# JWally/jsLPSolver

Hardware: AMD Instinct MI355X
Metric: simplex pivots/sec (higher is better)
Workload: dtype f64

## Files before the change

jslpsolver_amd/csrc/jslp_resident_pipe.hip.h:

```cpp
#pragma once

#ifdef JSLP_CHAOS_BUILD
#undef RT_MARK
#define RT_MARK(p)                                                                                                        \
    do {                                                                                                                  \
        if (F_TEST_LATE >= 2) {                                                                                     \
            const unsigned who_ = (R.epoch * 7u + (unsigned)(p) * 3u) % (unsigned)(THREADS / 64);                         \
            if (__builtin_amdgcn_readfirstlane((int)((unsigned)(threadIdx.x >> 6) == who_))) __builtin_amdgcn_s_sleep(100); \
            if (F_TEST_LATE >= 3 && (R.epoch + (unsigned)(p)) % 5u == (unsigned)blockIdx.x % 5u) __builtin_amdgcn_s_sleep(60); \
        }                                                                                                                 \
    } while (0)
#endif
#ifndef JSLP_PIPE_ROW_CHECKSUM
#define JSLP_PIPE_ROW_CHECKSUM 1
#endif
#ifndef JSLP_PIPE_K_BROADCAST
#define JSLP_PIPE_K_BROADCAST 1
#endif
#ifndef JSLP_PIPE_NORM_PUB
#define JSLP_PIPE_NORM_PUB 1
#endif
#ifndef JSLP_PIPE_ROW_CHECKSUM_MAXCPT
#define JSLP_PIPE_ROW_CHECKSUM_MAXCPT 4
#endif
#define JSLP_CK_K32(k) ((0x9E3779B1u * (unsigned)(2 * (k) + 1)) | 0x80000001u)
#define JSLP_CK_PAIR(CK, LO, HI, j)                                                                                               \
    do {                                                                                                                          \
        (CK) += (u64_t)(unsigned)(LO) * JSLP_CK_K32(2 * (j)) + (u64_t)(unsigned)((LO) >> 32) * JSLP_CK_K32(2 * (j) + 1);           \
        (CK) += (u64_t)(unsigned)(HI) * JSLP_CK_K32(2 * (j) + 2) + (u64_t)(unsigned)((HI) >> 32) * JSLP_CK_K32(2 * (j) + 3);       \
    } while (0)
#define JSLP_CK_TAGMIX(tag) ((u64_t)(tag) * 0xD6E8FEB86659FD93ull)
#ifndef JSLP_PIPE_POLL_MISSING_ONLY
#define JSLP_PIPE_POLL_MISSING_ONLY 1
#endif
#ifndef JSLP_PIPE_S_VIA_LDS
#define JSLP_PIPE_S_VIA_LDS 1
#endif
#define JSLP_PUB_SKEW 256
#ifndef JSLP_G16_STRIDE
#define JSLP_G16_STRIDE 64
#endif
#define JSLP_PIPE_KCHUNK 8

#define JSLP_HOST_ABORT_PERIOD 1024u
#ifndef JSLP_HOST_ABORT
#define JSLP_HOST_ABORT 1
#endif
#define JSLP_HOST_ABORT_FORCE_RETRY(SPINS) (JSLP_HOST_ABORT && (SPINS) == 0u && (epoch & (JSLP_HOST_ABORT_PERIOD - 1u)) == JSLP_HOST_ABORT_PERIOD - 1u && b == f.G - 1 && wv == HAWV)
#define JSLP_HOST_ABORT_IN_SPIN(SPINS, SWEPT)                                                                                     \
    if (JSLP_HOST_ABORT && (SPINS) == 1u && (epoch & (JSLP_HOST_ABORT_PERIOD - 1u)) == JSLP_HOST_ABORT_PERIOD - 1u && b == f.G - 1 && wv == HAWV) { \
        const unsigned* ha_ = *reinterpret_cast<const unsigned* const*>(reinterpret_cast<const char*>(f.cdev) + sizeof(Ctx));     \
        if (ha_ != nullptr && __hip_atomic_load(ha_, __ATOMIC_RELAXED, __HIP_MEMORY_SCOPE_SYSTEM) != 0u) {  \
            if (lane == 0) AG_STORE(f.abort_flag, 1u);                                                                            \
            (SWEPT) = false;                                                                                                      \
            break;                                                                                                                \
        }                                                                                                                         \
    }

__device__ __forceinline__ double readlane_f64(double x, int src_lane) {
    const long long b = __double_as_longlong(x);
    const unsigned lo = (unsigned)__builtin_amdgcn_readlane((int)(unsigned)b, src_lane);
    const unsigned hi = (unsigned)__builtin_amdgcn_readlane((int)(unsigned)((unsigned long long)b >> 32), src_lane);
    return __longlong_as_double((long long)(((unsigned long long)hi << 32) | lo));
}


static_assert(offsetof(RSmem, cycbits_tail) == offsetof(RSmem, lhist) + sizeof(int2) * JSLP_R_LHIST, "the filter runs from inside lhist into cycbits_tail");
static_assert((JSLP_R_LHIST - JSLP_PIPE_LHIST) * 8 + JSLP_R_CYCEXTRA * 4 == JSLP_PIPE_CYCBITS / 8, "filter size");
__device__ __forceinline__ unsigned* cyc_bits(RSmem& sm) { return reinterpret_cast<unsigned*>(&sm.lhist[JSLP_PIPE_LHIST]); }
__device__ __forceinline__ int cyc_pair_seen(RSmem& sm, int2 pair) {
    static_assert(JSLP_PIPE_CYCBITS == (1 << 19), "the hashes below yield 19 bits");
    unsigned* bits = cyc_bits(sm);
    const unsigned k = (unsigned)pair.x * 0x9E3779B1u ^ (unsigned)pair.y * 0x85EBCA6Bu;
    const unsigned h1 = k >> (32 - 19), h2 = (k * 0xC2B2AE35u + 0x27D4EB2Fu) >> (32 - 19);
    const unsigned o1 = bits[h1 >> 5], m1 = 1u << (h1 & 31u);
    bits[h1 >> 5] = o1 | m1;
    const unsigned o2 = bits[h2 >> 5], m2 = 1u << (h2 & 31u);
    bits[h2 >> 5] = o2 | m2;
    return ((o1 & m1) != 0u && (o2 & m2) != 0u) ? 1 : 0;
}
__device__ __forceinline__ bool cyc_suffix_is_square(const int2* lds, const int2* glob, int n, int2 last, Smem& red) {
    auto at = [&](int i) -> int2 { return i < JSLP_PIPE_LHIST ? lds[i] : glob[i]; };
    int found = 0;
    for (int L = 1 + threadIdx.x; 2 * L <= n; L += blockDim.x) {
        const int2 a = at(n - 1 - L);
        if (a.x != last.x || a.y != last.y) continue;
        bool eq = true;
        for (int i = 0; i < L - 1; i++) {
            const int2 x = at(n - 2 * L + i), y = at(n - L + i);
            if (x.x != y.x || x.y != y.y) { eq = false; break; }
        }
        if (eq) found = 1;
    }
    (void)red;
    return __syncthreads_or(found) != 0;
}

#define JSLP_WAVE_FOLD32(X, OP, ID)                                                                                              \
    do {                                                                                                                         \
        X = OP(X, __builtin_amdgcn_update_dpp((int)(ID), X, 0xB1, 0xf, 0xf, false));                                             \
        X = OP(X, __builtin_amdgcn_update_dpp((int)(ID), X, 0x4E, 0xf, 0xf, false));                                             \
        X = OP(X, __builtin_amdgcn_update_dpp((int)(ID), X, 0x141, 0xf, 0xf, false));                                            \
        X = OP(X, __builtin_amdgcn_update_dpp((int)(ID), X, 0x140, 0xf, 0xf, false));                                            \
        X = OP(X, __builtin_amdgcn_update_dpp((int)(ID), X, 0x142, 0xa, 0xf, false));                                            \
        X = OP(X, __builtin_amdgcn_update_dpp((int)(ID), X, 0x143, 0xc, 0xf, false));                                            \
        X = __builtin_amdgcn_readlane(X, 63);                                                                                    \
    } while (0)
__device__ __forceinline__ int jslp_add_i32(int a, int b) { return (int)((unsigned)a + (unsigned)b); }
__device__ __forceinline__ u64_t u64_wave_add_halves(u64_t x) {
    int lo = (int)(unsigned)x, hi = (int)(unsigned)(x >> 32);
    JSLP_WAVE_FOLD32(lo, jslp_add_i32, 0);
    JSLP_WAVE_FOLD32(hi, jslp_add_i32, 0);
    return (u64_t)(unsigned)lo | ((u64_t)(unsigned)hi << 32);
}
#define JSLP_CK_WAVE(CK) u64_wave_add_halves((CK) * (u64_t)(unsigned)(2 * tid + 1))

static_assert(offsetof(RSmem, part_r) % 8 == 0 && JSLP_F_MAXG / 64 >= 2, "winner and verdict are one aligned 8-byte word");
template <int CPT, int ROWS>
struct PipeDiet {
    static constexpr bool ONE_BARRIER = ROWS <= 8 && CPT <= 4;
    static constexpr bool RAW_ATOMICS = ROWS <= 8 && CPT <= 4;
};

__device__ __forceinline__ unsigned lds_offset(const void* p) { return (unsigned)(size_t)(__attribute__((address_space(3))) const void*)p; }
__device__ __forceinline__ void lds_max_u64_raw(u64_t* p, u64_t v) { asm volatile("ds_max_u64 %0, %1" : : "v"(lds_offset(p)), "v"(v) : "memory"); }
__device__ __forceinline__ void lds_min_i32_raw(int32_t* p, int v) { asm volatile("ds_min_i32 %0, %1" : : "v"(lds_offset(p)), "v"(v) : "memory"); }
__device__ __forceinline__ void lds_raw_drain() { asm volatile("s_waitcnt lgkmcnt(0)" : : : "memory"); }
template <bool ONE>
__device__ __forceinline__ void gather_post(RSmem& sm, int winner, bool swept) {
    if (ONE) *reinterpret_cast<int2*>(&sm.part_r[0]) = make_int2(winner, swept ? 1 : 0);
    else sm.part_r[0] = winner;
}
template <bool ONE>
__device__ __forceinline__ bool gather_close(RSmem& sm, bool swept, int* winner) {
    if (ONE) {
        __syncthreads();
        const int2 v = *reinterpret_cast<const int2*>(&sm.part_r[0]);
        *winner = v.x;
        return v.y != 0;
    }
    const bool ok = __syncthreads_and(swept ? 1 : 0) != 0;
    *winner = sm.part_r[0];
    return ok;
}

template <int THREADS, int CPT, bool UNR, bool RAW>
__device__ __forceinline__ int price_row_pipe(const double (&x)[CPT], int c0, const int (&pb)[CPT], const Ctx& c, RSmem& sm, int par,
                                              double* value, unsigned unr, int* neg, bool* claim) {
    const int tid = threadIdx.x, lane = tid & 63, wv = tid >> 6;
    double bv = c.precision;
    int bi = 0, bb = 0, bneg = 0;
#pragma unroll
    for (int j = 0; j < CPT; j++) {
        const int col = c0 + j;
        const bool isneg = UNR && ((unr >> j) & 1u) && x[j] < 0;
        const double val = isneg ? -x[j] : x[j];
        const bool ok = col >= 1 && col < c.W && val > c.precision;
        const bool take = ok && (bi == 0 || pb[j] < bb || (pb[j] == bb && val > bv));
        bv = take ? val : bv;
        bi = take ? col : bi;
        bb = take ? pb[j] : bb;
        bneg = take ? (isneg ? 1 : 0) : bneg;
    }
    {
        const unsigned long long m = __ballot(bi != 0);
        if (m != 0ull) {
            const int first = __ffsll((long long)m) - 1;
            const int wave_b = __builtin_amdgcn_readlane(bb, first);
            if (lane == 0) { if (RAW) lds_min_i32_raw(&sm.pw_batch[par], wave_b); else atomicMin(&sm.pw_batch[par], wave_b); }
        }
    }
    if (RAW) lds_raw_drain();
    __syncthreads();
    const int wb = sm.pw_batch[par];
    if (tid == THREADS - 1) { sm.pw_batch[par ^ 1] = 0x7fffffff; sm.pw_val[par ^ 1] = 0; sm.pw_col[par ^ 1] = 0x7fffffff; }
    *claim = false;
    if (wb == 0x7fffffff) return 0;
    const u64_t bits = (u64_t)__double_as_longlong(bv);
    const bool cand = bi != 0 && bb == wb;
    if (cand) { if (RAW) lds_max_u64_raw(&sm.pw_val[par], bits); else atomicMax(&sm.pw_val[par], bits); }
    if (RAW) lds_raw_drain();
    __syncthreads();
    const u64_t wvv = sm.pw_val[par];
    if (cand && bits == wvv) { if (RAW) lds_min_i32_raw(&sm.pw_col[par], bi); else atomicMin(&sm.pw_col[par], bi); }
    if (RAW) lds_raw_drain();
    __syncthreads();
    const int pcol = sm.pw_col[par];
    double v = __longlong_as_double((long long)wvv);
    if (UNR) {
        if (cand && bi == pcol) sm.pw_neg[par] = bneg;
        __syncthreads();
        *neg = sm.pw_neg[par];
        if (*neg) v = -v;
    }
    *value = v;
    *claim = wv == ((pcol / CPT) >> 6);
    return pcol;
}

#define JSLP_R_MAXOPT 3

template <int CPT>
__device__ __forceinline__ int price_optional_regs(const double (&x)[CPT], const double (&oo)[JSLP_R_MAXOPT][CPT], int c0, const Ctx& c, RSmem& sm) {
    const double precision = c.precision;
    for (int o = 0; o < c.n_opt && o < JSLP_R_MAXOPT; o++) {
        Cand best; best.v = precision; best.i = 0; best.b = 0;
#pragma unroll
        for (int j = 0; j < CPT; j++) {
            const int col = c0 + j;
            if (col < 1 || col >= c.W) continue;
            bool deferred = -precision < x[j] && x[j] < precision;
#pragma unroll
            for (int q = 0; q < JSLP_R_MAXOPT; q++) {
                if (q > o || !deferred) break;
                const double v = oo[q][j];
                if (q < o) { deferred = -precision < v && v < precision; continue; }
                if (-precision < v && v < precision) break;
                const bool take = v > best.v;
                best.v = take ? v : best.v;
                best.i = take ? col : best.i;
            }
        }
        const Cand e = block_reduce(best, PriceFirst(), sm.f.red);
        if (e.i != 0) return e.i;
    }
    return 0;
}

#define JSLP_PIPE_UPDATE_ROW(i)                                                                             \
    do {                                                                                                    \
        const int r_ = r_begin + (i);                                                                       \
        if (r_ >= r_end) break;                                                                             \
        if (r_ == 0) {                                                \
            _Pragma("unroll") for (int j = 0; j < CPT; j++) a[i][j] = r0[j];                                \
            break;                                                                                          \
        }                                                                                                   \
        if (r_ == pr_p) {                                                                                   \
            _Pragma("unroll") for (int j = 0; j < CPT; j++) a[i][j] = p[j];                                 \
            break;                                                                                          \
        }                                                                                                   \
        const double ki_ = kis[i];                                                                          \
        if (nonzero16(ki_)) {                                                                               \
            _Pragma("unroll") for (int j = 0; j < CPT; j++)                                                 \
                if ((nzm >> j) & 1u) a[i][j] = eliminate(a[i][j], ki_, p[j]);                               \
            if (has_pc_p) {                                                                                 \
                const double nv_ = sm.nv[i];                                                                \
                _Pragma("unroll") for (int j = 0; j < CPT; j++)                                             \
                    if (pc_p == c0 + j) a[i][j] = nv_;                                                      \
            }                                                                                               \
        }                                                                                                   \
    } while (0)

template <int CPT, int ROWS, bool OPT, bool XL>
struct PipeUpd {
    static constexpr bool UFAST = !XL && !OPT && ROWS <= 8 && CPT <= 4;
    static constexpr bool PUBTREE = UFAST && ROWS == 8;
    static constexpr unsigned ALL_ROWS = (unsigned)((1ull << ROWS) - 1ull);
    static __device__ __forceinline__ unsigned dead_rows(int live) { return ALL_ROWS & ~(unsigned)((1ull << max(0, min(ROWS, live))) - 1ull); }
};
#define JSLP_OPAQUE_SGPR(x) ({ int o_ = (x); asm volatile("" : "+s"(o_)); o_; })
#define JSLP_XL_UPDATE_PASS()                                                                                                     \
    do {                                                                                                                          \
                                                                                              \
        const double kl_ = lane < ROWS ? sm.colb[par_p][lane] : 0.0;                                                              \
        const unsigned km_ = (unsigned)__ballot(nonzero16(kl_));    \
         \
        if (UFAST) {                                                                                                              \
                  \
            double kb_[ROWS];                                                                                                     \
            _Pragma("unroll") for (int i = 0; i < ROWS; i++) kb_[i] = sm.colb[par_p][i];                                          \
            const int om_ = (int)(km_ | dead_rows), full_ = (int)ALL_ROWS;                                                        \
            if (om_ == full_) {                                                                                                   \
                _Pragma("unroll") for (int j = 0; j < CPT; j++) {                                                                 \
                    if ((nzm >> j) & 1u) {                                                                                        \
                        _Pragma("unroll") for (int i = 0; i < ROWS; i++) a[i][j] = eliminate(a[i][j], kb_[i], p[j]);              \
                    }                                                                                                             \
                }                                                                                                                 \
            }                                                                                                                     \
            if (JSLP_OPAQUE_SGPR(om_) != full_) {                                                                                 \
                _Pragma("unroll") for (int j = 0; j < CPT; j++) {                                                                 \
                    if ((nzm >> j) & 1u) {                                                                                        \
                        _Pragma("unroll") for (int i = 0; i < ROWS; i++)                                                          \
                            if (km_ & (1u << i)) a[i][j] = eliminate(a[i][j], kb_[i], p[j]);                                      \
                    }                                                                                                             \
                }                                                                                                                 \
            }                                                                                                                     \
        } else if (JSLP_PIPE_K_BROADCAST) {                                                                                       \
            _Pragma("unroll") for (int i0 = 0; i0 < ROWS; i0 += 8) {                                                              \
                double kb_[8];                                                                                                    \
                _Pragma("unroll") for (int i = 0; i < 8; i++) kb_[i] = (i0 + i < ROWS) ? sm.colb[par_p][i0 + i] : 0.0;            \
                _Pragma("unroll") for (int j = 0; j < CPT; j++) {                                                                 \
                    if ((nzm >> j) & 1u) {                                                                                        \
                        _Pragma("unroll") for (int i = 0; i < 8; i++)                                                             \
                            if (i0 + i < ROWS && (km_ & (1u << (i0 + i)))) a[i0 + i][j] = eliminate(a[i0 + i][j], kb_[i], p[j]);  \
                    }                                                                                                             \
                }                                                                                                                 \
            }                                                                                                                     \
        } else {                                                                                                                  \
        _Pragma("unroll") for (int j = 0; j < CPT; j++) {                                                                         \
            if ((nzm >> j) & 1u) {                                                                                                \
                _Pragma("unroll") for (int i = 0; i < ROWS; i++)                                                                  \
                    if (km_ & (1u << i)) a[i][j] = eliminate(a[i][j], readlane_f64(kl_, i), p[j]);                                \
            }                                                                                                                     \
        }                                                                                                                         \
        }                                                                                                                         \
        if (wv == ((pc_p / CPT) >> 6)) {          \
            const int ol_ = __builtin_amdgcn_readfirstlane((pc_p / CPT) & 63), js_ = __builtin_amdgcn_readfirstlane(pc_p % CPT);  \
             \
            const double nvl_ = lane < ROWS ? (NPUB ? -kl_ / quot_p : sm.nv[lane]) : 0.0;                                         \
            _Pragma("unroll") for (int j = 0; j < CPT; j++)                                                                       \
                if (js_ == j) {                                                                                                   \
                    _Pragma("unroll") for (int i = 0; i < ROWS; i++)                                                              \
                        if (km_ & (1u << i)) { const double nv_ = readlane_f64(nvl_, i); if (lane == ol_) a[i][j] = nv_; }        \
                }                                                                                                                 \
        }                                                                                                                         \
        {                                                                 \
            const int ip_ = __builtin_amdgcn_readfirstlane(pr_p - r_begin);                                                       \
            if (ip_ >= 0 && ip_ < ROWS) {                                                                                         \
                _Pragma("unroll") for (int i = 0; i < ROWS; i++)                                                                  \
                    if (i == JSLP_OPAQUE_SGPR(ip_)) { _Pragma("unroll") for (int j = 0; j < CPT; j++) a[i][j] = p[j]; }           \
            }                                                                                                                     \
        }                                                                                                                         \
        if (b == 0) { _Pragma("unroll") for (int j = 0; j < CPT; j++) a[0][j] = r0[j]; }    \
    } while (0)
#define JSLP_XL_PUBLISH_ROW(ROW)                                                                                                  \
    do {                                                                                                                          \
        const int ipub_ = __builtin_amdgcn_readfirstlane((ROW) - r_begin);                                                        \
        if (colok) {                                                                                                              \
            _Pragma("unroll") for (int i = 0; i < ROWS; i++)                                                                      \
                if (i == JSLP_OPAQUE_SGPR(ipub_)) {                                                                                                 \
                    const int off_ = par * pub_stride + (b * ld + c0) * 16;                                                       \
                    _Pragma("unroll") for (int j = 0; j < CPT; j++) {                                                             \
                        if (c0 + j >= ld) continue;                                                                               \
                        const u64_t d_ = (u64_t)__double_as_longlong(a[i][j]);                                                    \
                        v4u_t v_;                                                                                                 \
                        v_.x = (unsigned)d_; v_.y = tag; v_.z = (unsigned)(d_ >> 32); v_.w = tag;                                 \
                        __builtin_amdgcn_raw_buffer_store_b128(v_, rsrc_rows, off_ + j * 16, 0, ST_AUX);                          \
                    }                                                                                                             \
                }                                                                                                                 \
        }                                                                                                                         \
    } while (0)
#define JSLP_PUB_COPY(i) do { _Pragma("unroll") for (int j = 0; j < CPT; j++) { double t_ = a[i][j]; asm volatile("" : "+v"(t_)); cand_[j] = t_; } } while (0)
#define JSLP_PUBLISH_ROW_PLAIN(ROW)                                                                                               \
    do {                                                                                                                          \
        const int ipub_ = __builtin_amdgcn_readfirstlane((ROW) - r_begin);                                                        \
                     \
        const bool flag_first_ = CKS && __builtin_amdgcn_readfirstlane((int)(F_TEST_LATE == 2 && wv == 0)) != 0;                  \
        const bool torn_ = CKS && __builtin_amdgcn_readfirstlane((int)((F_TEST_LATE == 4 || F_TEST_LATE == 6) && wv == 0)) != 0;  \
        const bool early_lane_ = !torn_ || ((lane & 1) == (F_TEST_LATE == 6 ? 1 : 0));                                            \
        u64_t ck_ = 0;                                                                                                            \
        double cand_[CPT];                      \
        _Pragma("unroll") for (int j = 0; j < CPT; j++) cand_[j] = 0.0;                                                           \
        if (PUBTREE) {  \
            if (JSLP_OPAQUE_SGPR(ipub_) < 4) {                                                                                    \
                if (JSLP_OPAQUE_SGPR(ipub_) < 2) { if (JSLP_OPAQUE_SGPR(ipub_) == 0) JSLP_PUB_COPY(0); else if (JSLP_OPAQUE_SGPR(ipub_) == 1) JSLP_PUB_COPY(1); } \
                else { if (JSLP_OPAQUE_SGPR(ipub_) == 2) JSLP_PUB_COPY(2); else if (JSLP_OPAQUE_SGPR(ipub_) == 3) JSLP_PUB_COPY(3); } \
            } else {                                                                                                              \
                if (JSLP_OPAQUE_SGPR(ipub_) < 6) { if (JSLP_OPAQUE_SGPR(ipub_) == 4) JSLP_PUB_COPY(4); else if (JSLP_OPAQUE_SGPR(ipub_) == 5) JSLP_PUB_COPY(5); } \
                else { if (JSLP_OPAQUE_SGPR(ipub_) == 6) JSLP_PUB_COPY(6); else if (JSLP_OPAQUE_SGPR(ipub_) == 7) JSLP_PUB_COPY(7); } \
            }                                                                                                                     \
        } else                                                                                                                    \
        _Pragma("unroll") for (int i = 0; i < ROWS; i++)                                                                          \
            if (i == JSLP_OPAQUE_SGPR(ipub_)) {  \
                _Pragma("unroll") for (int j = 0; j < CPT; j++) { double t_ = a[i][j]; asm volatile("" : "+v"(t_)); cand_[j] = t_; }               \
            }                                                                                                                     \
        double quotc_ = 0.0, nv0c_ = 0.0;                                                                                         \
        if (NPUB) {                                                                                                               \
                         \
            quotc_ = sm.colb[par][ipub_];                                                                                         \
                                               \
            const bool holds_pc_ = __builtin_amdgcn_readfirstlane((int)(wv == ((pub_pc / CPT) >> 6))) != 0;                       \
            double rq_ = 0.0;                                                                                                     \
            if (holds_pc_) { rq_ = 1.0 / quotc_; nv0c_ = -pub_k0 / quotc_; }                                                      \
            _Pragma("unroll") for (int j = 0; j < CPT; j++) {                                                                     \
                const int col_ = c0 + j;                                                                                          \
                const double val_ = cand_[j];                                                                                     \
                double v_ = 0.0;                                                                                                  \
                if (col_ < W) {                                                                                                   \
                    const bool innz_ = nonzero16(val_);                                                                           \
                    v_ = innz_ ? val_ / quotc_ : 0.0;                                                                             \
                    if (col_ == pub_pc) v_ = rq_;                                                                                 \
                    if (innz_ && !nonzero16(v_) && v_ != 0.0) v_ = 0.0;  \
                }                                                                                                                 \
                cand_[j] = v_;                                                                                                    \
            }                                                                                                                     \
        }                                                                                                                         \
        const int off_ = PERM ? par * pub_stride + b * SLOT + lane_off : par * pub_stride + (b * ld + c0) * 8;                    \
        if (colok) {                                                                                                              \
            _Pragma("unroll") for (int j = 0; j < CPT; j += 2) {                                                                  \
                if (c0 + j >= ld) continue;                                                                                       \
                const u64_t lo_ = (u64_t)__double_as_longlong(cand_[j]), hi_ = (u64_t)__double_as_longlong(cand_[j + 1]);         \
                v4u_t v_;                                                                                                         \
                v_.x = (unsigned)lo_; v_.y = (unsigned)(lo_ >> 32); v_.z = (unsigned)hi_; v_.w = (unsigned)(hi_ >> 32);           \
                if (!flag_first_ && early_lane_) __builtin_amdgcn_raw_buffer_store_b128(v_, rsrc_rows, off_ + (j >> 1) * PAIR_STEP, 0, ST_AUX); \
                if (CKS) JSLP_CK_PAIR(ck_, lo_, hi_, j);                                                                          \
            }                                                                                                                     \
        }                                                                                                                         \
        if (CKS) { if (NPUB) JSLP_CKS_RAISE_REC(ck_, quotc_, nv0c_); else JSLP_CKS_RAISE_FLAG(ck_); }                              \
        if (flag_first_ || torn_) {                                                                                               \
            __builtin_amdgcn_s_sleep(127);                                                                                        \
            if (colok && (flag_first_ || !early_lane_)) {                                                                         \
                _Pragma("unroll") for (int j = 0; j < CPT; j += 2) {                                                              \
                    if (c0 + j >= ld) continue;                                                                                   \
                    const u64_t lo_ = (u64_t)__double_as_longlong(cand_[j]), hi_ = (u64_t)__double_as_longlong(cand_[j + 1]);     \
                    v4u_t v_;                                                                                                     \
                    v_.x = (unsigned)lo_; v_.y = (unsigned)(lo_ >> 32); v_.z = (unsigned)hi_; v_.w = (unsigned)(hi_ >> 32);       \
                    __builtin_amdgcn_raw_buffer_store_b128(v_, rsrc_rows, off_ + (j >> 1) * PAIR_STEP, 0, ST_AUX);                \
                }                                                                                                                 \
            }                                                                                                                     \
        }                                                                                                                         \
    } while (0)
#define JSLP_CKS_RAISE_FLAG(CK)                                                                                                   \
    do {                                                                                                                          \
        const u64_t x_ = JSLP_CK_WAVE(CK) ^ JSLP_CK_TAGMIX(tag);                                                                  \
        if (lane == 0) AG_STORE(f.rowflagc[par] + wv * JSLP_F_MAXG + b, x_);                                                      \
    } while (0)
#define JSLP_CK_QMIX(Q, NV) (((u64_t)__double_as_longlong(Q) * 0x9E3779B97F4A7C15ull) ^ ((u64_t)__double_as_longlong(NV) * 0xC2B2AE3D27D4EB4Full))
#define JSLP_REC_OFF(PAR, WV, B) (JSLP_R_REC_OFF + (((PAR) * JSLP_R_FLAGCOPIES + (WV)) * JSLP_F_MAXG + (B)) * JSLP_R_REC_BYTES)
#define JSLP_CKS_RAISE_REC(CK, Q, NV)                                                                                             \
    do {                                                                                                                          \
        const u64_t x_ = JSLP_CK_WAVE(CK) ^ JSLP_CK_TAGMIX(tag) ^ JSLP_CK_QMIX(Q, NV);                                            \
        if (lane == 0) {                                                                                                          \
            const u64_t qb_ = (u64_t)__double_as_longlong(Q), nb_ = (u64_t)__double_as_longlong(NV);                              \
            v4u_t r0_, r1_;                                                                                                       \
            r0_.x = (unsigned)x_; r0_.y = (unsigned)(x_ >> 32); r0_.z = (unsigned)qb_; r0_.w = (unsigned)(qb_ >> 32);             \
            r1_.x = (unsigned)nb_; r1_.y = (unsigned)(nb_ >> 32); r1_.z = tag; r1_.w = 0u;                                        \
            __builtin_amdgcn_raw_buffer_store_b128(r0_, rsrc_g16, JSLP_REC_OFF(par, wv, b), 0, ST_AUX);                           \
            __builtin_amdgcn_raw_buffer_store_b128(r1_, rsrc_g16, JSLP_REC_OFF(par, wv, b) + 16, 0, ST_AUX);                      \
        }                                                                                                                         \
    } while (0)
#define JSLP_CKS_ISSUE_LOOK()                                                                                                     \
    do {                                                                                                                          \
        if (__builtin_amdgcn_readfirstlane((int)((F_TEST_LATE & 1) != 0 && wv == 0))) __builtin_amdgcn_s_sleep(127);              \
        if (NPUB) {                                     \
            rec0_ = __builtin_amdgcn_raw_buffer_load_b128(rsrc_g16, JSLP_REC_OFF(par, wv, bw), 0, 16);                            \
            rec1_ = __builtin_amdgcn_raw_buffer_load_b128(rsrc_g16, JSLP_REC_OFF(par, wv, bw) + 16, 0, 16);                       \
        } else {                                                                                                                  \
            flag_ = AG_LOAD(f.rowflagc[par] + wv * JSLP_F_MAXG + bw);                                                             \
        }                                                                                                                         \
    } while (0)
#define JSLP_CKS_FETCH_ROW()                                                                                                      \
    do {                                                                                                                          \
        efetch += 1;                                                                                                              \
        unsigned spins_ = 0;                                                                                                      \
        const u64_t tmix_ = JSLP_CK_TAGMIX(tag);                                                                                  \
        u64_t flag_ = 0;                                                                                                          \
        v4u_t rec0_, rec1_;                                                                                                       \
        rec0_.x = rec0_.y = rec0_.z = rec0_.w = 0u; rec1_ = rec0_;                                                                \
        for (;;) {                                                                                                                \
            JSLP_CKS_ISSUE_LOOK();     \
            u64_t qm_ = 0;                                                                                                        \
            u64_t ck_ = 0;                                                                                                        \
            if (colok) {                                                                                                          \
                _Pragma("unroll") for (int j = 0; j < CPT; j += 2) {                                                              \
                    if (c0 + j >= ld) continue;                                                                                   \
                    const v4u_t v_ = __builtin_amdgcn_raw_buffer_load_b128(rsrc_rows, off_in + (j >> 1) * PAIR_STEP, 0, 16);  \
                    const u64_t lo_ = (u64_t)v_.x | ((u64_t)v_.y << 32), hi_ = (u64_t)v_.z | ((u64_t)v_.w << 32);                 \
                    pv[j] = __longlong_as_double((long long)lo_);                                                                 \
                    pv[j + 1] = __longlong_as_double((long long)hi_);                                                             \
                    JSLP_CK_PAIR(ck_, lo_, hi_, j);                                                           \
                }                                                                                                                 \
            }                                                                                                                     \
            if (NPUB) {                                                                                                           \
                flag_ = (u64_t)rec0_.x | ((u64_t)rec0_.y << 32);                                                                  \
                fq = __longlong_as_double((long long)((u64_t)rec0_.z | ((u64_t)rec0_.w << 32)));                                  \
                fnv = __longlong_as_double((long long)((u64_t)rec1_.x | ((u64_t)rec1_.y << 32)));                                 \
                qm_ = JSLP_CK_QMIX(fq, fnv);                                                                                      \
            }                                                                                                                     \
            const u64_t x_ = JSLP_CK_WAVE(ck_) ^ tmix_ ^ qm_;                                                                     \
            if (__builtin_amdgcn_readfirstlane((int)(x_ == flag_))) break;                                                        \
            JSLP_RT_RETRY();                                                                                                      \
            if (lane == 0) atomicAdd(f.abort_flag + 1, 1u);  \
            __builtin_amdgcn_s_sleep(1);                                                                                          \
            ++spins_;                                                                                                             \
            bool dead_ = false;                                                                                                   \
            if ((spins_ & 63u) == 0 && AG_LOAD(f.abort_flag) != 0u) dead_ = true;                                                 \
            if (spins_ > F_SPIN) { if (lane == 0) AG_STORE(f.abort_flag, 1u); dead_ = true; }                                     \
            if (dead_) { if (lane == 0) atomicMax(&sm.okbad, efetch); break; }                                                    \
        }                                                                                                                         \
    } while (0)
#ifdef JSLP_DEBUG_RESIDENT
#define JSLP_RT_RETRY() do { if (tid == 0) R.rt_retries += 1; } while (0)
#else
#define JSLP_RT_RETRY() do { } while (0)
#endif
#define JSLP_XL_FETCH_ROW(PCCOL, QUOT)                                                                                            \
    do {                                                                                                                          \
        efetch += 1;                                                                                                              \
        unsigned spins_ = 0;                                                                                                      \
        const int off_ = par * pub_stride + (bw * ld + c0) * 16;                                                                  \
        const int offq_ = par * pub_stride + (bw * ld + (PCCOL)) * 16;       \
        for (;;) {                                                                                                                \
            if (__builtin_amdgcn_readfirstlane((int)(F_TEST_LATE != 0 && wv == 0))) __builtin_amdgcn_s_sleep(127);          \
            bool ok_ = true;                                                                                                      \
            if (colok) {                                                                                                          \
                _Pragma("unroll") for (int j = 0; j < CPT; j++) {                                                                 \
                    if (c0 + j >= ld) continue;                                                                                   \
                    const v4u_t v_ = __builtin_amdgcn_raw_buffer_load_b128(rsrc_rows, off_ + j * 16, 0, 16);                      \
                    ok_ = ok_ && v_.y == tag && v_.w == tag;                                                                      \
                    pv[j] = __longlong_as_double((long long)((u64_t)v_.x | ((u64_t)v_.z << 32)));                                 \
                }                                                                                                                 \
            }                                                                                                                     \
            if ((PCCOL) > 0) {                                                                                                    \
                const v4u_t q_ = __builtin_amdgcn_raw_buffer_load_b128(rsrc_rows, offq_, 0, 16);                                  \
                ok_ = ok_ && q_.y == tag && q_.w == tag;                                                                          \
                (QUOT) = __longlong_as_double((long long)((u64_t)q_.x | ((u64_t)q_.z << 32)));                                    \
            }                                                                                                                     \
            if (__all(ok_)) break;                                                                                                \
            __builtin_amdgcn_s_sleep(1);                                                                                          \
            ++spins_;                                                                                                             \
            bool dead_ = false;                                                                                                   \
            if ((spins_ & 63u) == 0 && AG_LOAD(f.abort_flag) != 0u) dead_ = true;                                                 \
            if (spins_ > F_SPIN) { if (lane == 0) AG_STORE(f.abort_flag, 1u); dead_ = true; }                               \
            if (dead_) { if (lane == 0) atomicMax(&sm.okbad, efetch); break; }                                                    \
        }                                                                                                                         \
    } while (0)

#define JSLP_PIPE_COMMIT_GLOBAL_NOW()                                                                                             \
    do {                                                                                                                          \
        const Ctx& g_ = *f.cdev;                                                                                                  \
        g_.vibr[pr] = entering;                                                                                                   \
        g_.vibc[pc] = leaving;                                                                                                    \
        g_.rbv[entering] = pr;                                                                                                    \
        g_.rbv[leaving] = -1;                                                                                                     \
        g_.cbv[entering] = -1;                                                                                                    \
        g_.cbv[leaving] = pc;                                                                                                     \
        if (R.trace_n < g_.trace_cap) g_.trace[R.trace_n] = make_int2(pr, pc);                                                    \
    } while (0)
#define JSLP_PIPE_HIST_GLOBAL(PAIR)                                                                                               \
    do {                                                                                                                          \
        jslp_gi32_t* const h_ = (jslp_gi32_t*)jslp_uniform_ptr(sm.gp_hist) + 2 * R.hist_n;                                        \
        h_[0] = (PAIR).x; h_[1] = (PAIR).y;                                                                                       \
    } while (0)
#define JSLP_PIPE_SWAP_LDS_MAPS()                                                                                                 \
    do {                                                                                                                          \
        if (lpend && tid == THREADS - 64) {                                                                                       \
            const int leaving_ = sm.lvibr[pr_p], entering_ = sm.lvibc[pc_p];                                                      \
            sm.lvibr[pr_p] = entering_;                                                                                           \
            sm.lvibc[pc_p] = leaving_;                                                                                            \
            if (b == 0) { sm.cm_ent = entering_; sm.cm_leav = leaving_; }                                                         \
        }                                                                                                                         \
        lpend = false;                                                                                                            \
    } while (0)
__device__ __forceinline__ void* jslp_uniform_ptr(const void* p) {
    const unsigned long long b = (unsigned long long)p;
    const unsigned lo = (unsigned)__builtin_amdgcn_readfirstlane((int)(unsigned)b), hi = (unsigned)__builtin_amdgcn_readfirstlane((int)(unsigned)(b >> 32));
    return (void*)(((unsigned long long)hi << 32) | lo);
}
typedef __attribute__((address_space(1))) int32_t jslp_gi32_t;
#define JSLP_PIPE_COMMIT_GLOBAL()                                                                                                 \
    do {                                                                                                                          \
        if (cpend && tid == THREADS - 64 && b == 0) {                                                                             \
            const int ent_ = sm.cm_ent, leav_ = sm.cm_leav;  \
             \
            jslp_gi32_t* const vibr_ = (jslp_gi32_t*)jslp_uniform_ptr(sm.gp_vibr);                                               \
            jslp_gi32_t* const vibc_ = (jslp_gi32_t*)jslp_uniform_ptr(sm.gp_vibc);                                               \
            jslp_gi32_t* const rbv_ = (jslp_gi32_t*)jslp_uniform_ptr(sm.gp_rbv);                                                 \
            jslp_gi32_t* const cbv_ = (jslp_gi32_t*)jslp_uniform_ptr(sm.gp_cbv);                                                 \
            vibr_[pr_p] = ent_;                                                                                                   \
            vibc_[pc_p] = leav_;                                                                                                  \
            rbv_[ent_] = pr_p;                                                                                                    \
            rbv_[leav_] = -1;                                                                                                     \
            cbv_[ent_] = -1;                                                                                                      \
            cbv_[leav_] = pc_p;                                                                                                   \
            if (R.trace_n - 1 < sm.gp_trace_cap) {                                                                                \
                jslp_gi32_t* const tr_ = (jslp_gi32_t*)jslp_uniform_ptr(sm.gp_trace) + 2 * (R.trace_n - 1);                       \
                tr_[0] = pr_p; tr_[1] = pc_p;                                                                                     \
            }                                                                                                                     \
        }                                                                                                                         \
        cpend = false;                                                                                                            \
    } while (0)

template <int THREADS, int CPT, int ROWS, bool OPT, bool CHK, bool XL = false, bool UNR = false>
__device__ __forceinline__ void resident_phase2_pipe(const ResCtx& f, RSmem& sm, ResRegs<CPT, ROWS>& R, int it1_start, int it2_start,
                                                     const int (&pb)[CPT]) {
    const Ctx& c = f.c;
    const int tid = threadIdx.x, b = XL ? (int)(blockIdx.x / JSLP_XL_SPREAD) : (int)blockIdx.x, lane = tid & 63, wv = tid >> 6;
    constexpr int ST_AUX = XL ? 0 : 16;
    constexpr bool TAGGED = XL;
    constexpr bool CKS = !TAGGED && JSLP_PIPE_ROW_CHECKSUM != 0 && CPT <= JSLP_PIPE_ROW_CHECKSUM_MAXCPT;
    constexpr bool NPUB = CKS && !OPT && !XL && CPT <= 4 && ROWS <= 8 && JSLP_PIPE_NORM_PUB != 0;
    constexpr bool QDIRECT = TAGGED || NPUB;
    constexpr bool ONE_FOLD = ROWS <= 8 && CPT <= 4;
    constexpr bool S_LDS = XL || JSLP_PIPE_S_VIA_LDS != 0;
    constexpr bool UPD_NEW = XL || (CPT <= 4 && !(OPT && ROWS > 8));
    typedef PipeUpd<CPT, ROWS, OPT, XL> PU;
    constexpr bool UFAST = PU::UFAST, PUBTREE = PU::PUBTREE;
    static_assert(!UFAST || UPD_NEW, "the gate-free arm lives in JSLP_XL_UPDATE_PASS");
    constexpr unsigned ALL_ROWS = PU::ALL_ROWS;
    constexpr bool PERM = CPT >= 6;
    const int SLOT = PERM ? THREADS * CPT * 8 + JSLP_PUB_SKEW : f.c.ld * 8;
    constexpr int PAIR_STEP = PERM ? THREADS * 16 : 16;
    const int lane_off = PERM ? tid * 16 : tid * CPT * 8;
    constexpr bool CM_AT_N = OPT && ROWS > 8;
    constexpr int POLLWV = 1;
    constexpr int HAWV = POLLWV;
    static_assert(THREADS / 64 > POLLWV, "the polling wave exists");
    const int ld = c.ld, W = c.W;
    const double precision = c.precision;
    const int c0 = tid * CPT;
    const bool colok = c0 < ld;
    const int r_begin = b * f.rpb, r_end = min(f.H, r_begin + f.rpb);
    const unsigned dead_rows = PU::dead_rows(r_end - r_begin);
    (void)dead_rows; (void)ALL_ROWS;
    double (&a)[ROWS][CPT] = R.a;
    double (&r0)[CPT] = R.r0;
    typedef unsigned int v4u_t __attribute__((ext_vector_type(4)));
    const int pub_stride = (int)((const char*)f.rows_pub[1] - (const char*)f.rows_pub[0]);
    const auto rsrc_rows = __builtin_amdgcn_make_buffer_rsrc(f.rows_pub[0], 0, pub_stride + (TAGGED ? f.G * ld * 16 : f.G * (CPT >= 6 ? THREADS * CPT * 8 + JSLP_PUB_SKEW : ld * 8)), 0x00020000);
    const auto rsrc_g16 = __builtin_amdgcn_make_buffer_rsrc(f.gran16, 0, JSLP_R_REC_OFF + JSLP_R_REC_WORDS * 8, 0x00020000);
#ifdef JSLP_DEBUG_RESIDENT
    u64_t (&rt_acc)[8] = R.rt_acc;
    u64_t& rt_prev = R.rt_prev;
#endif

    double p[CPT];
    unsigned nzm = 0;
    int pr_p = 0, pc_p = 0, par_p = 0;
    double quot_p = 1.0;
    bool pend = false;
    bool cpend = false;
    bool lpend = false;
#pragma unroll
    for (int j = 0; j < CPT; j++) p[j] = 0.0;
    int okslot = 0;
    unsigned& efetch = R.efetch;


    if (tid == 0) sm.cyc_filter_on = R.hist_n == 0 ? 1 : 0;
    for (int i = tid; i < JSLP_PIPE_CYCBITS / 32; i += THREADS) cyc_bits(sm)[i] = 0u;
    if (tid == 0) {
#pragma unroll
        for (int i = 0; i < ROWS; i++) sm.rhsb[i] = a[i][0];
        for (int q = 0; q < 2; q++) { sm.pw_batch[q] = 0x7fffffff; sm.pw_val[q] = 0; sm.pw_col[q] = 0x7fffffff; sm.pw_neg[q] = 0; }
    }
    __syncthreads();

    while (R.end_code == 0) {
        const bool has_pc_p = pend && colok && pc_p >= c0 && pc_p < c0 + CPT;
        if ((R.it1 - it1_start) + (R.it2 - it2_start) >= F_ITERS) { R.end_code = 4; break; }
        if ((CHK && c.check_cycles) && !(R.hist_n < (f.hist_all ? JSLP_PIPE_GHIST : JSLP_PIPE_LHIST) && R.hist_n < c.hist_cap)) { R.end_code = 8; break; }
        const unsigned epoch = R.epoch;
        const int par = epoch & 1;
        const unsigned tag = epoch + 1;
        if (F_TEST_ABORT >= 0 && (int)epoch == F_TEST_ABORT && b == f.G - 1) {
            if (tid == 0) AG_STORE(f.abort_flag, 1u);
            R.end_code = 5;
            break;
        }
        RT_MARK(7);
        double k0 = 0.0;
        int pc;
        bool claim = false;
        {
            int neg_now = 0;
            RT_STAMP(5);
            pc = price_row_pipe<THREADS, CPT, UNR, PipeDiet<CPT, ROWS>::RAW_ATOMICS>(r0, c0, pb, c, sm, par, &k0, R.unr, &neg_now, &claim);
            RT_STAMP(6);
            JSLP_PIPE_SWAP_LDS_MAPS();
            if (UNR) R.neg = neg_now;
        }
        bool opt_enter = false;
        if (OPT && pc == 0 && c.n_opt > 0) {
            pc = price_optional_regs<CPT>(r0, R.oo, c0, c, sm);
            if (pc != 0) {
                opt_enter = true;
                if (colok && pc >= c0 && pc < c0 + CPT) {
#pragma unroll
                    for (int j = 0; j < CPT; j++)
                        if (pc == c0 + j) sm.xq[0] = r0[j];
                }
                __syncthreads();
                k0 = sm.xq[0];
            }
        }
        if (QDIRECT && !OPT && efetch != 0u && sm.okbad == efetch) { R.end_code = 5; pend = false; break; }
        if (pc == 0) { R.end_code = 1; break; }
        RT_MARK(6);
        if (OPT && opt_enter) claim = wv == ((pc / CPT) >> 6);
        if (claim) {
            const int ol = __builtin_amdgcn_readfirstlane((pc / CPT) & 63);
            const int jsel = __builtin_amdgcn_readfirstlane(pc % CPT);
            double x = 0.0, pj = 0.0;
            unsigned nzj = 0;
#pragma unroll
            for (int j = 0; j < CPT; j++)
                if (jsel == j) {
                    if (S_LDS) {
                        if (lane == ol) {
#pragma unroll
                            for (int i = 0; i < ROWS; i++) sm.quo[i] = a[i][j];
                        }
                    } else {
#pragma unroll
                        for (int i = 0; i < ROWS; i++) {
                            const double xi = readlane_f64(a[i][j], ol);
                            x = lane == i ? xi : x;
                        }
                    }
                    pj = readlane_f64(p[j], ol);
                    nzj = ((unsigned)__builtin_amdgcn_readlane((int)nzm, ol) >> j) & 1u;
                }
            if (S_LDS) {
                __builtin_amdgcn_wave_barrier();
                __builtin_amdgcn_s_waitcnt(0xc07f);
                x = lane < ROWS ? sm.quo[lane] : 0.0;
            }
            const int r = r_begin + lane;
            double colv = 0.0;
            int kind = 0;
            double quo = 0.0;
            if (lane < ROWS) {
                colv = x;
                if (pend) {
                    const double ki = sm.colb[par_p][lane];
                    if (r == pr_p) colv = pj;
                    else if (r != 0 && r < r_end && nonzero16(ki)) {
                        if (__builtin_amdgcn_readfirstlane(pc_p) == __builtin_amdgcn_readfirstlane(pc)) colv = NPUB ? -ki / quot_p : sm.nv[lane];
                        else colv = nzj ? eliminate(x, ki, pj) : x;
                    }
                }
                sm.colb[par][lane] = colv;
                const double rhs = sm.rhsb[lane];
                if (r >= 1 && r < r_end && !(-precision < colv && colv < precision)) {
                    if (colv > 0 && precision > rhs && rhs > -precision) kind = 1;
                    else { quo = (UNR && R.neg) ? -rhs / colv : rhs / colv; kind = quo > precision && quo < INFINITY ? 2 : 0; }
                }
            }
            static_assert(ROWS <= 32, "the summary's DPP folds cover two 16-lane rows");
            int brdeg = ONE_FOLD ? 0x7fffffff : (kind == 1 ? r : 0x7fffffff);
            if (!ONE_FOLD) {
            brdeg = min(brdeg, __builtin_amdgcn_update_dpp(brdeg, brdeg, 0xB1, 0xf, 0xf, false));
            brdeg = min(brdeg, __builtin_amdgcn_update_dpp(brdeg, brdeg, 0x4E, 0xf, 0xf, false));
            brdeg = min(brdeg, __builtin_amdgcn_update_dpp(brdeg, brdeg, 0x141, 0xf, 0xf, false));
            if (ROWS > 8) brdeg = min(brdeg, __builtin_amdgcn_update_dpp(brdeg, brdeg, 0x140, 0xf, 0xf, false));
            brdeg = ROWS > 16 ? min(__builtin_amdgcn_readlane(brdeg, 0), __builtin_amdgcn_readlane(brdeg, 16))
                              : __builtin_amdgcn_readlane(brdeg, 0);
            }
            KI bk;
            if (ONE_FOLD) {
                bk.k = kind == 2 ? (u64_t)__double_as_longlong(quo) : (kind == 1 ? 0ull : KI_NONE_KEY);
                bk.i = kind != 0 ? r : 0x7fffffff;
            } else {
                bk.k = kind == 2 ? (u64_t)__double_as_longlong(quo) : KI_NONE_KEY;
                bk.i = kind == 2 ? r : 0x7fffffff;
            }
            bk.pad = 0;
            bk = ki_min(bk, ki_dpp<0xB1>(bk));
            bk = ki_min(bk, ki_dpp<0x4E>(bk));
            bk = ki_min(bk, ki_dpp<0x141>(bk));
            if (ROWS > 8) bk = ki_min(bk, ki_dpp<0x140>(bk));
            bk = ROWS > 16 ? ki_min(ki_readlane(bk, 0), ki_readlane(bk, 16)) : ki_readlane(bk, 0);
            if (lane == 0) {
                const bool deg = ONE_FOLD ? bk.k == 0ull : brdeg != 0x7fffffff;
                if (ONE_FOLD) brdeg = bk.i;
                const bool have = bk.k != KI_NONE_KEY;
                const int row = deg ? brdeg : (have ? bk.i : 0);
                const u64_t qb = (deg || !have) ? 0ull : bk.k;
                v4u_t g;
                g.x = (unsigned)qb;
                g.y = tag;
                g.z = (unsigned)(qb >> 32);
                g.w = ((tag & 0xffffu) << 16) | (deg ? 0x8000u : 0u) | (unsigned)row;
                __builtin_amdgcn_raw_buffer_store_b128(g, rsrc_g16, (par * JSLP_F_MAXG + b) * JSLP_G16_STRIDE, 0, ST_AUX);
                sm.pubrow = row;
            }
        }
        __syncthreads();
        const int pubrow = sm.pubrow;
        if (!CM_AT_N) JSLP_PIPE_COMMIT_GLOBAL();
        RT_STAMP(0);
        const double pub_k0 = k0;
        const int pub_pc = pc;
        (void)pub_k0; (void)pub_pc;
        RT_MARK(0);
        bool swept = true;
        const bool poller = wv == POLLWV;
        v4u_t g;
        g.x = 0; g.y = tag; g.z = 0; g.w = (tag & 0xffffu) << 16;
        if (UPD_NEW) {
            if (pend) JSLP_XL_UPDATE_PASS();
            if (pubrow != 0) {
                if (TAGGED) JSLP_XL_PUBLISH_ROW(pubrow);
                else JSLP_PUBLISH_ROW_PLAIN(pubrow);
            }
        } else {
        u64_t ck = 0;
        const bool flag_first_o = CKS && __builtin_amdgcn_readfirstlane((int)(F_TEST_LATE == 2 && wv == 0)) != 0;
        const bool torn_o = CKS && __builtin_amdgcn_readfirstlane((int)((F_TEST_LATE == 4 || F_TEST_LATE == 6) && wv == 0)) != 0;
        const bool early_lane_o = !torn_o || ((lane & 1) == (F_TEST_LATE == 6 ? 1 : 0));
#pragma unroll
        for (int i0 = 0; i0 < ROWS; i0 += JSLP_PIPE_KCHUNK) {
            double kis[ROWS];
#pragma unroll
            for (int i = i0; i < i0 + JSLP_PIPE_KCHUNK && i < ROWS; i++) kis[i] = sm.colb[par_p][i];
#pragma unroll
            for (int i = i0; i < i0 + JSLP_PIPE_KCHUNK && i < ROWS; i++) {
                if (pend) JSLP_PIPE_UPDATE_ROW(i);
                if (pubrow != 0 && r_begin + i == pubrow && colok) {
                    const int off = PERM ? par * pub_stride + b * SLOT + lane_off : par * pub_stride + (b * ld + c0) * 8;
#pragma unroll
                    for (int j = 0; j < CPT; j += 2) {
                        if (c0 + j >= ld) continue;
                        const u64_t lo = (u64_t)__double_as_longlong(a[i][j]), hi = (u64_t)__double_as_longlong(a[i][j + 1]);
                        v4u_t v;
                        v.x = (unsigned)lo; v.y = (unsigned)(lo >> 32); v.z = (unsigned)hi; v.w = (unsigned)(hi >> 32);
                        if (!flag_first_o && early_lane_o) __builtin_amdgcn_raw_buffer_store_b128(v, rsrc_rows, off + (j >> 1) * PAIR_STEP, 0, ST_AUX);
                        if (CKS) JSLP_CK_PAIR(ck, lo, hi, j);
                    }
                }
            }
        }
        if (CKS && pubrow != 0) JSLP_CKS_RAISE_FLAG(ck);
        if (CKS && pubrow != 0 && (flag_first_o || torn_o)) {
            __builtin_amdgcn_s_sleep(127);
            const int ipub_o = __builtin_amdgcn_readfirstlane(pubrow - r_begin);
            if (colok && (flag_first_o || !early_lane_o)) {
#pragma unroll
                for (int i = 0; i < ROWS; i++)
                    if (i == JSLP_OPAQUE_SGPR(ipub_o)) {
                        const int off = PERM ? par * pub_stride + b * SLOT + lane_off : par * pub_stride + (b * ld + c0) * 8;
#pragma unroll
                        for (int j = 0; j < CPT; j += 2) {
                            if (c0 + j >= ld) continue;
                            const u64_t lo = (u64_t)__double_as_longlong(a[i][j]), hi = (u64_t)__double_as_longlong(a[i][j + 1]);
                            v4u_t v;
                            v.x = (unsigned)lo; v.y = (unsigned)(lo >> 32); v.z = (unsigned)hi; v.w = (unsigned)(hi >> 32);
                            __builtin_amdgcn_raw_buffer_store_b128(v, rsrc_rows, off + (j >> 1) * PAIR_STEP, 0, ST_AUX);
                        }
                    }
            }
        }
        }
        pend = false;
        RT_STAMP(1);
        RT_MARK(2);
        if (poller) {
            unsigned spins = 0;
            v4u_t gq[JSLP_F_MAXG / 64];
#if JSLP_PIPE_POLL_MISSING_ONLY
            unsigned have = 0;
#pragma unroll
            for (int q = 0; q < JSLP_F_MAXG / 64; q++) {
                gq[q] = g;
                if (lane + 64 * q >= f.G) have |= 1u << q;
            }
#endif
            for (;;) {
                bool ok = true;
#if JSLP_PIPE_POLL_MISSING_ONLY
#pragma unroll
                for (int q = 0; q < JSLP_F_MAXG / 64; q++)
                    if (!((have >> q) & 1u)) gq[q] = __builtin_amdgcn_raw_buffer_load_b128(rsrc_g16, (par * JSLP_F_MAXG + lane + 64 * q) * JSLP_G16_STRIDE, 0, 16);
#pragma unroll
                for (int q = 0; q < JSLP_F_MAXG / 64; q++)
                    if (gq[q].y == tag && (gq[q].w >> 16) == (tag & 0xffffu)) have |= 1u << q;
                ok = have == (1u << (JSLP_F_MAXG / 64)) - 1u;
#else
#pragma unroll
                for (int q = 0; q < JSLP_F_MAXG / 64; q++) {
                    gq[q] = g;
                    if (lane + 64 * q < f.G) gq[q] = __builtin_amdgcn_raw_buffer_load_b128(rsrc_g16, (par * JSLP_F_MAXG + lane + 64 * q) * JSLP_G16_STRIDE, 0, 16);
                }
#pragma unroll
                for (int q = 0; q < JSLP_F_MAXG / 64; q++) ok = ok && gq[q].y == tag && (gq[q].w >> 16) == (tag & 0xffffu);
#endif
                if (__all(ok) && !JSLP_HOST_ABORT_FORCE_RETRY(spins)) break;
                __builtin_amdgcn_s_sleep(1);
                ++spins;
                JSLP_HOST_ABORT_IN_SPIN(spins, swept);
                if ((spins & 63u) == 0 && AG_LOAD(f.abort_flag) != 0u) { swept = false; break; }
                if (spins > F_SPIN) { if (lane == 0) AG_STORE(f.abort_flag, 1u); swept = false; break; }
            }
            int rdeg = 0x7fffffff;
            KI x = ki_none();
#pragma unroll
            for (int q = 0; q < JSLP_F_MAXG / 64; q++) {
                const int row = (int)(gq[q].w & 0x7fffu);
                const bool deg = (gq[q].w & 0x8000u) != 0u;
                if (!ONE_FOLD && deg && row != 0) rdeg = min(rdeg, row);
                KI y;
                const bool cand = ONE_FOLD ? row != 0 : !deg && row != 0;
                y.k = cand ? ((u64_t)gq[q].x | ((u64_t)gq[q].z << 32)) : KI_NONE_KEY;
                y.i = cand ? row : 0x7fffffff;
                y.pad = 0;
                x = ki_min(x, y);
            }
            if (!ONE_FOLD) {
            rdeg = min(rdeg, __builtin_amdgcn_update_dpp(rdeg, rdeg, 0xB1, 0xf, 0xf, false));
            rdeg = min(rdeg, __builtin_amdgcn_update_dpp(rdeg, rdeg, 0x4E, 0xf, 0xf, false));
            rdeg = min(rdeg, __builtin_amdgcn_update_dpp(rdeg, rdeg, 0x141, 0xf, 0xf, false));
            rdeg = min(rdeg, __builtin_amdgcn_update_dpp(rdeg, rdeg, 0x140, 0xf, 0xf, false));
            rdeg = min(min(__builtin_amdgcn_readlane(rdeg, 0), __builtin_amdgcn_readlane(rdeg, 16)),
                       min(__builtin_amdgcn_readlane(rdeg, 32), __builtin_amdgcn_readlane(rdeg, 48)));
            }
            x = ki_wave_min(x);
            if (lane == 0) { sm.part_k[0] = x.k; gather_post<PipeDiet<CPT, ROWS>::ONE_BARRIER>(sm, x.k == KI_NONE_KEY ? 0 : x.i, swept); if (!ONE_FOLD) sm.part_rdeg[0] = rdeg; }
        }
        RT_STAMP(2);
        RT_MARK(1);
        if (!TAGGED && !CKS) asm volatile("s_waitcnt vmcnt(0)" ::: "memory");
        int wr;
        if (!gather_close<PipeDiet<CPT, ROWS>::ONE_BARRIER>(sm, swept, &wr)) { R.end_code = 5; break; }
        RT_STAMP(3);
        RT_MARK(3);
        int pr = 0, stop = 0;
        {
            const int wrdeg = ONE_FOLD ? 0x7fffffff : sm.part_rdeg[0];
            if (wrdeg != 0x7fffffff) pr = wrdeg;
            else if (wr != 0) pr = wr;
            else stop = 3;
        }
        if (!stop && (CHK && c.check_cycles)) {
            if (tid == 0) {
                const int2 pair = make_int2(sm.lvibr[pr], sm.lvibc[pc]);
                if (R.hist_n < JSLP_PIPE_LHIST) sm.lhist[R.hist_n] = pair;
                if (f.hist_all) f.hist_all[(size_t)b * JSLP_PIPE_GHIST + R.hist_n] = pair;
                if (b == 0) JSLP_PIPE_HIST_GLOBAL(pair);
                sm.cyc_need = sm.cyc_filter_on ? cyc_pair_seen(sm, pair) : 1;
            }
            __syncthreads();
            R.hist_n += 1;
            if (sm.cyc_need != 0) {
                if (cyc_suffix_is_square(sm.lhist, f.hist_all ? f.hist_all + (size_t)b * JSLP_PIPE_GHIST : nullptr, R.hist_n, make_int2(sm.lvibr[pr], sm.lvibc[pc]), sm.f.red)) stop = 1;
            }
        }
        if (stop == 3) { R.end_code = 2; R.unbounded_col = pc; break; }
        if (stop == 1) { R.end_code = 3; break; }
        const bool leaving_unr = UNR && sm.lunr[sm.lvibr[pr]] != 0;
        const int bw = pr / f.rpb;
        if (!TAGGED && !CKS && bw == b) {
            if (tid < THREADS / 64) {
                if (XL) {
                    *reinterpret_cast<volatile u64_t*>(f.rowflagc[par] + tid * JSLP_F_MAXG + b) = (u64_t)tag;
                } else {
                    __builtin_amdgcn_fence(__ATOMIC_RELEASE, "agent");
                    AG_STORE(f.rowflagc[par] + tid * JSLP_F_MAXG + b, (u64_t)tag);
                }
            }
        }
        const int off_in = PERM ? par * pub_stride + bw * SLOT + lane_off : par * pub_stride + (bw * ld + c0) * 8;
        const bool has_pc = colok && pc >= c0 && pc < c0 + CPT;
        double pv[CPT];
#pragma unroll
        for (int j = 0; j < CPT; j++) pv[j] = 0.0;
        double quot = 0.0;
        double fq = 0.0, fnv = 0.0;
        double ook[JSLP_R_MAXOPT];
#pragma unroll
        for (int o = 0; o < JSLP_R_MAXOPT; o++) ook[o] = 0.0;
        {
            if (TAGGED) {
                JSLP_XL_FETCH_ROW(pc, quot);
            } else if (CKS) {
                JSLP_CKS_FETCH_ROW();
            } else {
            efetch += 1;
            unsigned spins = 0;
            for (;;) {
                if (__builtin_amdgcn_readfirstlane((int)(F_TEST_LATE != 0 && wv == 0))) __builtin_amdgcn_s_sleep(127);
// ... 638 lines not shown
```

Baseline: 223,800.

## Fold pricing batch and value into one packed LDS max key

For small geometries (ROWS<=8, CPT<=2), pricing row selection packs the batch index and the top 58 bits of the value into a single 64-bit key for one ds_max_u64 round. A second ds_max_u32 round then resolves the low value bits and the column. This replaces the former three-round reduction (batch min, value max, column) and removes a barrier from the per-pivot critical path. It relies on batch indices staying below 128 and column indices fitting in 16 bits, which static_asserts check. Tie-breaking changes: among equal values the lowest column now wins via the inverted column field.

```diff
diff --git a/jslpsolver_amd/csrc/jslp_resident_pipe.hip.h b/jslpsolver_amd/csrc/jslp_resident_pipe.hip.h
--- a/jslpsolver_amd/csrc/jslp_resident_pipe.hip.h
+++ b/jslpsolver_amd/csrc/jslp_resident_pipe.hip.h
@@ -120,11 +120,13 @@
 struct PipeDiet {
     static constexpr bool ONE_BARRIER = ROWS <= 8 && CPT <= 4;
     static constexpr bool RAW_ATOMICS = ROWS <= 8 && CPT <= 4;
+    static constexpr bool TWO_ROUNDS = ROWS <= 8 && CPT <= 2;
 };
 
 __device__ __forceinline__ unsigned lds_offset(const void* p) { return (unsigned)(size_t)(__attribute__((address_space(3))) const void*)p; }
 __device__ __forceinline__ void lds_max_u64_raw(u64_t* p, u64_t v) { asm volatile("ds_max_u64 %0, %1" : : "v"(lds_offset(p)), "v"(v) : "memory"); }
 __device__ __forceinline__ void lds_min_i32_raw(int32_t* p, int v) { asm volatile("ds_min_i32 %0, %1" : : "v"(lds_offset(p)), "v"(v) : "memory"); }
+__device__ __forceinline__ void lds_max_u32_raw(unsigned* p, unsigned v) { asm volatile("ds_max_u32 %0, %1" : : "v"(lds_offset(p)), "v"(v) : "memory"); }
 __device__ __forceinline__ void lds_raw_drain() { asm volatile("s_waitcnt lgkmcnt(0)" : : : "memory"); }
 template <bool ONE>
 __device__ __forceinline__ void gather_post(RSmem& sm, int winner, bool swept) {
@@ -144,7 +146,9 @@
     return ok;
 }
 
-template <int THREADS, int CPT, bool UNR, bool RAW>
+#define JSLP_PW_BATCH_MAX 127
+#define JSLP_PW_BATCH_SMALLEST 50
+template <int THREADS, int CPT, bool UNR, bool RAW, bool TWO>
 __device__ __forceinline__ int price_row_pipe(const double (&x)[CPT], int c0, const int (&pb)[CPT], const Ctx& c, RSmem& sm, int par,
                                               double* value, unsigned unr, int* neg, bool* claim) {
     const int tid = threadIdx.x, lane = tid & 63, wv = tid >> 6;
@@ -161,6 +165,36 @@
         bi = take ? col : bi;
         bb = take ? pb[j] : bb;
         bneg = take ? (isneg ? 1 : 0) : bneg;
+    }
+    if (TWO) {
+        static_assert(!TWO || RAW, "the two rounds are the lanes' own ds_max_u64 / ds_max_u32");
+        static_assert(!TWO || (THREADS * CPT - 1) / JSLP_PW_BATCH_SMALLEST <= JSLP_PW_BATCH_MAX, "more than 128 pricing batches: this geometry keeps the three-round form");
+        static_assert(!TWO || THREADS * CPT <= 0xffff, "the second key's column field: 16 bits");
+        const u64_t bits = (u64_t)__double_as_longlong(bv);
+        const u64_t key1 = ((u64_t)(unsigned)(JSLP_PW_BATCH_MAX - bb) << 57) | (bits >> 6);
+        if (bi != 0) lds_max_u64_raw(&sm.pw_val[par], key1);
+        lds_raw_drain();
+        __syncthreads();
+        const u64_t w1 = sm.pw_val[par];
+        if (tid == THREADS - 1) { sm.pw_val[par ^ 1] = 0; sm.pw_col[par ^ 1] = 0; }
+        *claim = false;
+        if (w1 == 0ull) return 0;
+        const bool cand = bi != 0 && key1 == w1;
+        if (cand) lds_max_u32_raw(reinterpret_cast<unsigned*>(&sm.pw_col[par]), (((unsigned)bits & 63u) << 16) | (0xffffu - (unsigned)bi));
+        lds_raw_drain();
+        __syncthreads();
+        const unsigned w2 = (unsigned)sm.pw_col[par];
+        const int pcol = (int)(0xffffu - (w2 & 0xffffu));
+        double v = __longlong_as_double((long long)(((w1 & ((1ull << 57) - 1ull)) << 6) | (u64_t)(w2 >> 16)));
+        if (UNR) {
+            if (cand && bi == pcol) sm.pw_neg[par] = bneg;
+            __syncthreads();
+            *neg = sm.pw_neg[par];
+            if (*neg) v = -v;
+        }
+        *value = v;
+        *claim = wv == ((pcol / CPT) >> 6);
+        return pcol;
     }
     {
         const unsigned long long m = __ballot(bi != 0);
@@ -632,7 +666,7 @@
     if (tid == 0) {
 #pragma unroll
         for (int i = 0; i < ROWS; i++) sm.rhsb[i] = a[i][0];
-        for (int q = 0; q < 2; q++) { sm.pw_batch[q] = 0x7fffffff; sm.pw_val[q] = 0; sm.pw_col[q] = 0x7fffffff; sm.pw_neg[q] = 0; }
+        for (int q = 0; q < 2; q++) { sm.pw_batch[q] = 0x7fffffff; sm.pw_val[q] = 0; sm.pw_col[q] = PipeDiet<CPT, ROWS>::TWO_ROUNDS ? 0 : 0x7fffffff; sm.pw_neg[q] = 0; }
     }
     __syncthreads();
 
@@ -655,7 +689,7 @@
         {
             int neg_now = 0;
             RT_STAMP(5);
-            pc = price_row_pipe<THREADS, CPT, UNR, PipeDiet<CPT, ROWS>::RAW_ATOMICS>(r0, c0, pb, c, sm, par, &k0, R.unr, &neg_now, &claim);
+            pc = price_row_pipe<THREADS, CPT, UNR, PipeDiet<CPT, ROWS>::RAW_ATOMICS, PipeDiet<CPT, ROWS>::TWO_ROUNDS>(r0, c0, pb, c, sm, par, &k0, R.unr, &neg_now, &claim);
             RT_STAMP(6);
             JSLP_PIPE_SWAP_LDS_MAPS();
             if (UNR) R.neg = neg_now;
```

New measurement: 229,400 (median of 6 runs). 1.03x the previous value.
